# mit-han-lab/pvcnn

Hardware: AMD Instinct MI355X
Metric: point-clouds/sec fwd+bwd, PVCNN S3DIS N=4096 R=32 (higher is better)
Workload: dtype f32 (fp32 tensors, fp32 accumulate; Conv3d fwd / bwd-data / bwd-weight and the large SharedMLP fwd / bwd-data / bwd-weight products as power-of-two scaled fp16 hi+lo splits, 3 partial products on fp16 MFMA, max rel err vs fp64 1e-6 <= the fp32-MFMA kernels'; PVCNN_CONV_MATH=fp32 PVCNN_PW_MATH=fp32 s; 1 GPU; PVCNN (1xC) S3DIS fwd+bwd+Adam, B=16/GPU N=4096 R=32/16 fp32; global_batch=16, points=4096, parallelism=dp1, gradient_bytes=10289972, step_mode=graph, rccl_ranks=0, gradient_buckets=2

## Files before the change

### include/pvcnn_hip.h

```cpp
#ifndef PVCNN_HIP_H_
#define PVCNN_HIP_H_

#include <stddef.h>
#include <stdint.h>

#ifdef __cplusplus
extern "C" {
#endif

#if defined(__GNUC__)
#define PVCNN_API __attribute__((visibility("default")))
#else
#define PVCNN_API
#endif

#define PVCNN_ABI_VERSION 15
#define PVCNN_OK 0
#define PVCNN_ERR_INVALID_ARGUMENT (-1)

PVCNN_API int pvcnn_version(void);
PVCNN_API const char *pvcnn_last_error_string(void);

PVCNN_API int pvcnn_voxel_coords(const float *coords, int B, int N, int R, int normalize, float eps, float *norm_coords,
                       int32_t *vox_coords, void *stream);

PVCNN_API int pvcnn_voxel_coords_tail(const float *coords, long coords_batch_stride, const float *mean, const float *radius,
                            int B, int N, int R, float eps, float *norm_coords, int32_t *vox_coords, void *stream);

PVCNN_API size_t pvcnn_avg_voxelize_fwd_workspace_bytes(int B, int C, int N, int R);
PVCNN_API int pvcnn_avg_voxelize_fwd(const float *feat, const int32_t *coords, int B, int C, int N, int R,
                           float *out, int32_t *ind, int32_t *cnt, void *workspace,
                           size_t workspace_bytes, void *stream);
PVCNN_API int pvcnn_avg_voxelize_bwd(const float *grad_y, const int32_t *ind, const int32_t *cnt, int B,
                           int C, int N, int S, float *grad_x, void *stream);

PVCNN_API int pvcnn_trilinear_devox_fwd(const float *coords, const float *feat, int B, int C, int N, int R,
                              int is_training, int32_t *inds, float *wgts, float *outs,
                              void *stream);
PVCNN_API size_t pvcnn_trilinear_devox_bwd_workspace_bytes(int B, int C, int N, int R);
PVCNN_API int pvcnn_trilinear_devox_bwd(const float *grad_y, const int32_t *inds, const float *wgts, int B,
                              int C, int N, int R, float *grad_x, void *workspace,
                              size_t workspace_bytes, void *stream);

PVCNN_API size_t pvcnn_avg_voxelize_plan_bytes(int B, int N, int R);
PVCNN_API size_t pvcnn_avg_voxelize_plan_scratch_bytes(int B, int N, int R);
PVCNN_API int pvcnn_avg_voxelize_plan(const int32_t *coords, int B, int N, int R, int32_t *ind, int32_t *cnt, void *plan,
                            size_t plan_bytes, void *scratch, size_t scratch_bytes, void *stream);
PVCNN_API size_t pvcnn_pvconv_plans_scratch_bytes(int B, int N, int R);
PVCNN_API int pvcnn_pvconv_plans(const int32_t *vox_coords, const float *norm_coords, int B, int N, int R, int32_t *ind, int32_t *cnt,
                                 void *vox_plan, size_t vox_plan_bytes, void *devox_bwd_plan, size_t devox_bwd_plan_bytes,
                                 void *scratch, size_t scratch_bytes, void *stream);
PVCNN_API int pvcnn_avg_voxelize_apply(const float *feat, const void *plan, size_t plan_bytes, int B, int C, int N, int R,
                             float *out, void *stream);
PVCNN_API size_t pvcnn_trilinear_devox_bwd_plan_bytes(int B, int N, int R);
PVCNN_API size_t pvcnn_trilinear_devox_bwd_plan_scratch_bytes(int B, int N, int R);
PVCNN_API int pvcnn_trilinear_devox_bwd_plan(const int32_t *inds, const float *wgts, int B, int N, int R, void *plan,
                                   size_t plan_bytes, void *scratch, size_t scratch_bytes, void *stream);
PVCNN_API int pvcnn_trilinear_devox_bwd_apply(const float *grad_y, long grad_y_batch_stride, const void *plan, size_t plan_bytes,
                                    int B, int C, int N, int R, float *grad_x, void *stream);

PVCNN_API int pvcnn_ball_query(const float *centers, const float *points, int B, int N, int M, float radius,
                     int U, int32_t *out, void *stream);

PVCNN_API int pvcnn_grouping_fwd(const float *features, const int32_t *indices, int B, int C, int N, int M,
                       int U, float *out, void *stream);
PVCNN_API size_t pvcnn_grouping_bwd_workspace_bytes(int B, int C, int N, int M, int U);
PVCNN_API int pvcnn_grouping_bwd(const float *grad_y, const int32_t *indices, int B, int C, int N, int M,
                       int U, float *grad_x, void *workspace, size_t workspace_bytes, void *stream);
PVCNN_API int pvcnn_gather_fwd(const float *features, const int32_t *indices, int B, int C, int N, int M,
                     float *out, void *stream);
PVCNN_API size_t pvcnn_gather_bwd_workspace_bytes(int B, int C, int N, int M);
PVCNN_API int pvcnn_gather_bwd(const float *grad_y, const int32_t *indices, int B, int C, int N, int M,
                     float *grad_x, void *workspace, size_t workspace_bytes, void *stream);

#define PVCNN_FPS_MAX_RESIDENT_POINTS 16384
PVCNN_API int pvcnn_fps(const float *coords, int B, int N, int M, float *distances, int32_t *indices,
              void *stream);

PVCNN_API int pvcnn_mask_select(const uint8_t *mask, int B, int N, int M, const int32_t *choices, const int64_t *seed,
                      int32_t *selected, int32_t *count, void *stream);

PVCNN_API size_t pvcnn_batch_lds_bytes(int N, int max_n);
PVCNN_API int pvcnn_batch_s3dis(const float *rows, const void *labels, int label_bytes, const int64_t *offsets, long long W, int max_n,
                      const int64_t *order, long long order_len, const int64_t *cursor, int B, int N, int C_out,
// ... 202 lines not shown
```

### pvcnn_amd/__init__.py

```python
import importlib
import sys

__version__ = '0.1.0'

_DROPIN_SUBMODULES = (
    'ball_query', 'frustum', 'loss', 'pointnet', 'pvconv', 'se', 'shared_mlp', 'voxelization',
    'functional', 'functional.backend', 'functional.ball_query', 'functional.devoxelization',
    'functional.grouping', 'functional.interpolatation', 'functional.loss', 'functional.sampling',
    'functional.voxelization',
)


def install_dropin(name='modules'):
    impl = importlib.import_module('pvcnn_amd.modules')
    sys.modules[name] = impl
    for sub in _DROPIN_SUBMODULES:
        sys.modules[f'{name}.{sub}'] = importlib.import_module(f'pvcnn_amd.modules.{sub}')
    return impl


_ADOPTED = {}


def _adopted_class(cls, forward, extra=None):
# ... 24 lines not shown
    from .modules import SharedMLP

    def is_head(seq):
        kids = list(seq)
        return (len(kids) >= 2 and isinstance(kids[0], SharedMLP) and isinstance(kids[-1], (nn.Conv1d, SharedMLP))
                and all(isinstance(k, (SharedMLP, nn.Dropout, nn.Conv1d)) for k in kids))

    def take(module, donor_forward, extra=None):
        if type(module).forward is not donor_forward:
            module.__class__ = _adopted_class(type(module), donor_forward, extra)

    for m in model.modules():
        if type(m) is nn.Sequential and is_head(m):
            m.__class__ = _adopted_class(nn.Sequential, _classify_forward)
    has = lambda obj, *names: all(hasattr(obj, a) for a in names)
    if has(model, 'inst_seg_net', 'center_reg_net', 'box_est_net'):
        seg, ctr, box = model.inst_seg_net, model.center_reg_net, model.box_est_net
        if has(seg, 'point_features', 'cloud_features', 'classifier', 'in_channels'):
            take(seg, workload._FrustumSegmentation.forward)
        if has(ctr, 'features', 'regression'):
            take(ctr, workload._CloudRegressor.forward, {'_head_attr': 'regression', '_coords_tuple': False})
        if has(box, 'features', 'classifier'):
            take(box, workload._CloudRegressor.forward, {'_head_attr': 'classifier', '_coords_tuple': True})
        return model
    donor = None
    if has(model, 'sa_layers', 'fp_layers', 'classifier'):
        donor = workload.PVCNN2
    elif has(model, 'point_features', 'classifier', 'num_shapes', 'in_channels') and isinstance(model.point_features, nn.ModuleList):
        donor = workload.PVCNNShapeNet
    elif has(model, 'point_features', 'cloud_features', 'classifier') and isinstance(model.point_features, nn.ModuleList):
        donor = workload.PVCNN
    if donor is not None:
        take(model, donor.forward)
    return model
```

### pvcnn_amd/_lib.py

```python
import ctypes
import functools
import os

import torch

_CSRC = os.path.join(os.path.dirname(os.path.abspath(__file__)), 'csrc')
LIB_PATH = os.path.join(_CSRC, 'libpvcnn_hip.so')
ABI_VERSION = 15

_vp, _i, _f, _sz, _l = ctypes.c_void_p, ctypes.c_int, ctypes.c_float, ctypes.c_size_t, ctypes.c_long
_ll = ctypes.c_longlong

SIGNATURES = {
    'pvcnn_version': (_i, []),
    'pvcnn_last_error_string': (ctypes.c_char_p, []),
    'pvcnn_voxel_coords': (_i, [_vp, _i, _i, _i, _i, _f, _vp, _vp, _vp]),
    'pvcnn_voxel_coords_tail': (_i, [_vp, ctypes.c_long, _vp, _vp, _i, _i, _i, _f, _vp, _vp, _vp]),
    'pvcnn_avg_voxelize_fwd_workspace_bytes': (_sz, [_i, _i, _i, _i]),
    'pvcnn_avg_voxelize_fwd': (_i, [_vp, _vp, _i, _i, _i, _i, _vp, _vp, _vp, _vp, _sz, _vp]),
    'pvcnn_avg_voxelize_bwd': (_i, [_vp, _vp, _vp, _i, _i, _i, _i, _vp, _vp]),
    'pvcnn_trilinear_devox_fwd': (_i, [_vp, _vp, _i, _i, _i, _i, _i, _vp, _vp, _vp, _vp]),
    'pvcnn_trilinear_devox_bwd_workspace_bytes': (_sz, [_i, _i, _i, _i]),
    'pvcnn_trilinear_devox_bwd': (_i, [_vp, _vp, _vp, _i, _i, _i, _i, _vp, _vp, _sz, _vp]),
    'pvcnn_avg_voxelize_plan_bytes': (_sz, [_i, _i, _i]),
    'pvcnn_avg_voxelize_plan_scratch_bytes': (_sz, [_i, _i, _i]),
    'pvcnn_avg_voxelize_plan': (_i, [_vp, _i, _i, _i, _vp, _vp, _vp, _sz, _vp, _sz, _vp]),
    'pvcnn_avg_voxelize_apply': (_i, [_vp, _vp, _sz, _i, _i, _i, _i, _vp, _vp]),
    'pvcnn_pvconv_plans_scratch_bytes': (_sz, [_i, _i, _i]),
    'pvcnn_pvconv_plans': (_i, [_vp, _vp, _i, _i, _i, _vp, _vp, _vp, _sz, _vp, _sz, _vp, _sz, _vp]),
    'pvcnn_trilinear_devox_bwd_plan_bytes': (_sz, [_i, _i, _i]),
    'pvcnn_trilinear_devox_bwd_plan_scratch_bytes': (_sz, [_i, _i, _i]),
    'pvcnn_trilinear_devox_bwd_plan': (_i, [_vp, _vp, _i, _i, _i, _vp, _sz, _vp, _sz, _vp]),
    'pvcnn_trilinear_devox_bwd_apply': (_i, [_vp, ctypes.c_long, _vp, _sz, _i, _i, _i, _i, _vp, _vp]),
    'pvcnn_ball_query': (_i, [_vp, _vp, _i, _i, _i, _f, _i, _vp, _vp]),
    'pvcnn_grouping_fwd': (_i, [_vp, _vp, _i, _i, _i, _i, _i, _vp, _vp]),
    'pvcnn_grouping_bwd_workspace_bytes': (_sz, [_i, _i, _i, _i, _i]),
    'pvcnn_grouping_bwd': (_i, [_vp, _vp, _i, _i, _i, _i, _i, _vp, _vp, _sz, _vp]),
    'pvcnn_gather_fwd': (_i, [_vp, _vp, _i, _i, _i, _i, _vp, _vp]),
    'pvcnn_gather_bwd_workspace_bytes': (_sz, [_i, _i, _i, _i]),
    'pvcnn_gather_bwd': (_i, [_vp, _vp, _i, _i, _i, _i, _vp, _vp, _sz, _vp]),
    'pvcnn_fps': (_i, [_vp, _i, _i, _i, _vp, _vp, _vp]),
    'pvcnn_mask_select': (_i, [_vp, _i, _i, _i, _vp, _vp, _vp, _vp, _vp]),
    'pvcnn_three_nn_interp_fwd': (_i, [_vp, _vp, _vp, _i, _i, _i, _i, _vp, _vp, _vp, _vp]),
    'pvcnn_three_nn_interp_bwd_workspace_bytes': (_sz, [_i, _i, _i, _i]),
    'pvcnn_three_nn_interp_bwd': (_i, [_vp, _vp, _vp, _i, _i, _i, _i, _vp, _vp, _sz, _vp]),
    'pvcnn_conv3d_weight_transform': (_i, [_vp, _i, _i, _i, _vp, _vp]),
    'pvcnn_conv3d_fwd': (_i, [_vp, _vp, _vp, _i, _i, _i, _i, _vp, _vp]),
    'pvcnn_conv3d_bwd_weight_workspace_bytes': (_sz, [_i, _i, _i, _i]),
    'pvcnn_conv3d_bwd_weight': (_i, [_vp, _vp, _i, _i, _i, _i, _vp, _vp, _vp, _sz, _vp]),
    'pvcnn_conv3d_weight_split_bytes': (_sz, [_i, _i, _i, _i]),
    'pvcnn_conv3d_weight_split': (_i, [_vp, _i, _i, _i, _i, _vp, _vp]),
    'pvcnn_conv3d_weight_split_pair': (_i, [_vp, _i, _i, _vp, _vp, _vp]),
    'pvcnn_conv3d_fwd_split_stats_parts': (_sz, [_i, _i, _i, _i]),
    'pvcnn_conv3d_fwd_split_route': (_i, [_i, _i, _i, _i, _i]),
    'pvcnn_absmax_bits': (_i, [_vp, _sz, _vp, _vp]),
    'pvcnn_absmax_tiles_count': (_sz, [_i, ctypes.c_long, _i]),
    'pvcnn_absmax_tiles': (_i, [_vp, _i, _i, ctypes.c_long, _i, _vp, _vp, _vp]),
    'pvcnn_conv3d_bwd_weight_f16_workspace_bytes': (_sz, [_i, _i, _i, _i]),
    'pvcnn_conv3d_bwd_weight_f16': (_i, [_vp, _vp, _vp, _i, _vp, _i, _i, _i, _i, _i, _vp, _vp, _vp, _sz, _vp]),
    'pvcnn_conv3d_fwd_split': (_i, [_vp, _vp, _vp, _i, _i, _i, _i, _i, _vp, _i, _vp, _vp, _vp]),
    'pvcnn_pwconv_transpose': (_i, [_vp, _i, _i, _vp, _vp]),
    'pvcnn_pwconv_fwd': (_i, [_vp, _vp, _i, _vp, _i, _i, _i, _i, _vp, _vp]),
# ... 113 lines not shown
```

### pvcnn_amd/csrc/csr.h

```cpp
#pragma once
#include <algorithm>

#include "slab.h"

namespace pvcnn {

constexpr int kCsrThreads = 1024;
constexpr int kCsrMaxTargets = 1 << 20;
constexpr int kCsrMaxRange = 14336;

__host__ __device__ __forceinline__ int pad32(int v) { return v + (v >> 5); }
__host__ __device__ __forceinline__ int start_stride(int L) { return (L + 1 + 3) & ~3; }

constexpr int kTileTargets = 4096;
constexpr int kTileThreads = 1024;
__host__ __device__ inline int order_stride(int L) { return ceil_div(L, kTileTargets) * kTileTargets; }

constexpr int kGroupSlack = 256;
__host__ __device__ inline long entw_range_base(int start_t0, int r) { return 2L * start_t0 + (long)r * (kTileTargets / kWave) * kGroupSlack; }
__host__ __device__ inline long entw_stride(int L, long E) { return 2L * E + (long)ceil_div(L, kTileTargets) * (kTileTargets / kWave) * kGroupSlack; }

struct CsrPlan {
  int32_t *start;
  int2 *ent;
// ... 716 lines not shown
template <class EP1, class EP2>
int launch_csr_prep_pair(const EP1 &ep1, long E1_, int32_t *cnt1, void *plan1, size_t plan1_bytes, const EP2 &ep2, long E2_, void *plan2,
                         size_t plan2_bytes, int B, int L, void *scratch, size_t scratch_bytes, hipStream_t s, const char *what) {
  const int E1 = (int)E1_, E2 = (int)E2_;
  if (B == 0) return 0;
  const size_t s1 = csr_prep_scratch_bytes(B, E1), s2 = csr_prep_scratch_bytes(B, E2);
  if (!plan1 || !plan2 || plan1_bytes < CsrPlan::bytes(B, L, E1) || plan2_bytes < CsrPlan::bytes(B, L, E2) || !aligned16(plan1) ||
      !aligned16(plan2) || !scratch || !aligned16(scratch) || scratch_bytes < s1 + s2) {
    set_error("%s: plans / scratch missing, misaligned or too small (%zu, %zu, %zu bytes needed)", what, CsrPlan::bytes(B, L, E1),
              CsrPlan::bytes(B, L, E2), s1 + s2);
    return PVCNN_ERR_INVALID_ARGUMENT;
  }
  CsrPlan p1, p2;
  p1.carve(plan1, B, L, E1);
  p2.carve(plan2, B, L, E2);
  const int total = std::max(2, std::min(16, kNumCU / std::max(B, 1)));
  const int cap1 = std::max(1, total / 4);
  const CsrSplit sp1 = csr_split(B, L, E1, cap1), sp2 = csr_split(B, L, E2, std::max(1, total - cap1));
  const size_t prep_lds = ((size_t)kCsrCoarse * 2 + 4 + 32 + 4 + 3 * kCsrList + std::max(sp1.HP, sp2.HP)) * sizeof(int);
  auto k = csr_prep_pair_kernel<EP1, EP2>;
  if (int e = enable_big_lds(k, prep_lds)) { set_error("%s: LDS attribute: %d", what, e); return e; }
  char *sc = static_cast<char *>(scratch);
  hipLaunchKernelGGL(k, dim3(sp1.P + sp2.P, B), dim3(kCsrThreads), prep_lds, s, ep1, E1, sp1, cnt1, p1.start, reinterpret_cast<int32_t *>(sc),
                     p1.ent, ep2, E2, sp2, p2.start, reinterpret_cast<int32_t *>(sc + s1), p2.ent, L);
  if (int e = check_launch(what)) return e;
  const CsrPlanRef r1{p1.start, p1.ent, p1.order, p1.seg, p1.gofs, p1.entw, E1}, r2{p2.start, p2.ent, p2.order, p2.seg, p2.gofs, p2.entw, E2};
  const int nr = ceil_div(L, kTileTargets), nblk = order_stride(L) / 256;
  hipLaunchKernelGGL(csr_order_pair_kernel, dim3(2 * nr, B), dim3(kTileThreads), 0, s, r1, r2, L, nr);
  if (int e = check_launch(what)) return e;
  hipLaunchKernelGGL(csr_interleave_pair_kernel, dim3(2 * nblk, B), dim3(256), 0, s, r1, r2, L, nblk);
  return check_launch(what);
}

inline int launch_csr_apply(const float *src, const void *plan, size_t plan_bytes, float *dst, int B, int C, int L, int J, long E_,
                            hipStream_t s, const char *what, long src_bstride = 0) {
  if (src_bstride <= 0) src_bstride = (long)C * J;
  const int E = (int)E_;
  if (B == 0 || C == 0) return 0;
  if (!plan || plan_bytes < CsrPlan::bytes(B, L, E) || !aligned16(plan)) {
    set_error("%s: plan missing, misaligned or too small (%zu bytes needed)", what, CsrPlan::bytes(B, L, E));
    return PVCNN_ERR_INVALID_ARGUMENT;
  }
  CsrPlan pl;
  pl.carve(const_cast<void *>(plan), B, L, E);
  const int JP = (J + 3) & ~3;
  int G = 0;
  for (int cand = 4; cand >= 1; cand >>= 1)
    if ((size_t)cand * (JP + kTileTargets) * sizeof(float) <= (size_t)kLdsBytesPerCU) { G = cand; break; }
  const size_t row = (size_t)J * sizeof(float);
  int GS = 1;
  if (row > 0 && row <= 64 * 1024) {
    GS = (int)std::min<size_t>(8, (64 * 1024) / row);
    while (GS > 1 && (long)B * ceil_div(C, GS) < 2L * kNumCU) GS >>= 1;
    if (GS >= 8) GS = 8; else if (GS >= 4) GS = 4; else if (GS >= 2) GS = 2; else GS = 1;
  }
  const bool very_sparse = (long)E * 4 <= (long)L && row > 0 && row <= (size_t)kLdsBytesPerCU && (long)B * ceil_div(C, GS) >= kNumCU;
  if (G > 0 && J > 0 && !very_sparse) {
    while (G > 1 && G / 2 >= C) G >>= 1;
    const int nr = ceil_div(L, kTileTargets), slabs = ceil_div(C, G);
    int nsplit = 1;
    while (nsplit < nr && (long)B * slabs * nsplit < kNumCU) nsplit <<= 1;
    nsplit = std::min(nsplit, nr);
    const size_t lds = (size_t)G * (JP + kTileTargets) * sizeof(float);
    const dim3 grid(slabs, nsplit, B);
#define PVCNN_TILE(GV)                                                                                                   \
  do {                                                                                                                   \
// ... 38 lines not shown
```

### pvcnn_amd/csrc/voxelize.hip

```cpp
#include <algorithm>

#include "csr.h"

namespace pvcnn {

__global__ __launch_bounds__(256) void vox_stats_atomic_kernel(const int32_t *__restrict__ coords, int N,
                                                               int R, int S, int32_t *__restrict__ ind,
                                                               int32_t *__restrict__ cnt) {
  const int b = blockIdx.y, i = blockIdx.x * 256 + threadIdx.x;
  if (i >= N) return;
  const int32_t *co = coords + (size_t)b * 3 * N;
  int v = co[i] * R * R + co[i + N] * R + co[i + 2 * N];
  v = min(max(v, 0), S - 1);
  ind[(size_t)b * N + i] = v;
  atomicAdd(cnt + (size_t)b * S + v, 1);
}

__global__ __launch_bounds__(256) void vox_scatter_atomic_kernel(
    const float *__restrict__ feat, const int32_t *__restrict__ ind, const int32_t *__restrict__ cnt, int C,
    int N, int S, int CT, float *__restrict__ out) {
  const int b = blockIdx.z, i = blockIdx.x * 256 + threadIdx.x;
  if (i >= N) return;
  const int pos = ind[(size_t)b * N + i];
  const int cur = cnt[(size_t)b * S + pos];
// ... 198 lines not shown
  PVCNN_REQUIRE(B >= 0 && N >= 0 && R > 0, "negative size");
  PVCNN_REQUIRE((long)R * R * R <= 0x7fffffffL / 4, "resolution too large");
  const int S = R * R * R;
  if (B == 0) return 0;
  PVCNN_REQUIRE(csr_supported(S, N), "grid too large for a plan: use pvcnn_avg_voxelize_fwd");
  PVCNN_REQUIRE(cnt && (ind || N == 0) && (coords || N == 0), "null pointer");
  PVCNN_REQUIRE(B <= 65535, "batch > 65535");
  VoxelEntries ep{coords, ind, N, R, S};
  return launch_csr_prep(ep, B, S, N, cnt, plan, plan_bytes, scratch, scratch_bytes, static_cast<hipStream_t>(stream),
                         "avg_voxelize_plan");
}

extern "C" size_t pvcnn_pvconv_plans_scratch_bytes(int B, int N, int R) {
  if (B <= 0 || N < 0 || R <= 0) return 0;
  return csr_prep_scratch_bytes(B, N) + csr_prep_scratch_bytes(B, 8L * N);
}

extern "C" int pvcnn_pvconv_plans(const int32_t *vox_coords, const float *norm_coords, int B, int N, int R, int32_t *ind, int32_t *cnt,
                                  void *vox_plan, size_t vox_plan_bytes, void *devox_bwd_plan, size_t devox_bwd_plan_bytes, void *scratch,
                                  size_t scratch_bytes, void *stream) {
  PVCNN_REQUIRE(B >= 0 && N > 0 && R > 0, "bad size");
  PVCNN_REQUIRE((long)R * R * R <= 0x7fffffffL / 4, "resolution too large");
  const int S = R * R * R;
  if (B == 0) return 0;
  PVCNN_REQUIRE(csr_supported(S, 8L * N), "grid too large for a plan: use the one-shot calls");
  PVCNN_REQUIRE(cnt && ind && vox_coords && norm_coords, "null pointer");
  PVCNN_REQUIRE(B <= 65535, "batch > 65535");
  VoxelEntries e1{vox_coords, ind, N, R, S};
  CoordTapEntries e2{norm_coords, N, R, R * R, S};
  return launch_csr_prep_pair(e1, N, cnt, vox_plan, vox_plan_bytes, e2, 8L * N, devox_bwd_plan, devox_bwd_plan_bytes, B, S,
                              scratch, scratch_bytes, static_cast<hipStream_t>(stream), "pvconv_plans");
}

extern "C" int pvcnn_avg_voxelize_apply(const float *feat, const void *plan, size_t plan_bytes, int B, int C, int N, int R,
                                        float *out, void *stream) {
  PVCNN_REQUIRE(B >= 0 && C >= 0 && N >= 0 && R > 0, "negative size");
  PVCNN_REQUIRE((long)R * R * R <= 0x7fffffffL / 4, "resolution too large");
  if (B == 0 || C == 0) return 0;
  PVCNN_REQUIRE(out && (feat || N == 0), "null pointer");
  PVCNN_REQUIRE(B <= 65535, "batch > 65535");
  const int S = R * R * R;
  return launch_csr_apply(feat, plan, plan_bytes, out, B, C, S, N, N, static_cast<hipStream_t>(stream),
                          "avg_voxelize_apply");
}
```

### pvcnn_amd/modules/functional/backend.py

```python
import ctypes
import os

import torch

from ... import _lib
from . import _cache

__all__ = ['_backend']


def _dev(t, name):
    if not t.is_cuda:
        raise RuntimeError(f'{name} must be a CUDA (HIP) tensor -- the PVConv hot path has no CPU implementation')


def _f32(t, name):
    _dev(t, name)
    if not t.is_contiguous():
        raise RuntimeError(f'{name} must be a contiguous tensor')
    if t.dtype != torch.float32:
        raise RuntimeError(f'{name} must be a float tensor')


def _f32_rows(t, name):
# ... 364 lines not shown
        vp.r, vp.n, vp.b = r, n, b
        vp.ind = torch.empty((b, n), dtype=torch.int32, device=dev)
        vp.cnt = torch.empty((b, r * r * r), dtype=torch.int32, device=dev)
        vp.plan = torch.empty((nbytes,), dtype=torch.uint8, device=dev)
        scratch = self._scratch(self.lib.pvcnn_avg_voxelize_plan_scratch_bytes(b, n, r), dev)
        with _Launch(coords) as s:
            _lib.check(self.lib.pvcnn_avg_voxelize_plan(_p(coords), b, n, r, _p(vp.ind), _p(vp.cnt), _p(vp.plan), vp.plan.numel(),
                                                        _p(scratch), scratch.numel(), s), 'avg_voxelize_plan')
        return vp

    has_pvconv_plans = os.environ.get('PVCNN_PAIR_PLANS', '1') != '0'

    def pvconv_plans(self, vox_coords, norm_coords, resolution):
        _i32(vox_coords, 'vox_coords'); _f32(norm_coords, 'norm_coords')
        _shape(vox_coords.dim() == 3 and vox_coords.shape[1] == 3 and tuple(norm_coords.shape) == tuple(vox_coords.shape),
               'pvconv_plans: vox_coords / norm_coords (B,3,N) expected')
        b, _, n = vox_coords.shape
        r = int(resolution)
        vbytes, dbytes = self.lib.pvcnn_avg_voxelize_plan_bytes(b, n, r), self.lib.pvcnn_trilinear_devox_bwd_plan_bytes(b, n, r)
        if vbytes == 0 or dbytes == 0 or n == 0:
            return None
        dev = vox_coords.device
        vp = self.VoxelPlan()
        vp.r, vp.n, vp.b = r, n, b
        vp.ind = torch.empty((b, n), dtype=torch.int32, device=dev)
        vp.cnt = torch.empty((b, r * r * r), dtype=torch.int32, device=dev)
        vp.plan = torch.empty((vbytes,), dtype=torch.uint8, device=dev)
        dplan = torch.empty((dbytes,), dtype=torch.uint8, device=dev)
        scratch = self._scratch(self.lib.pvcnn_pvconv_plans_scratch_bytes(b, n, r), dev)
        with _Launch(vox_coords) as s:
            _lib.check(self.lib.pvcnn_pvconv_plans(_p(vox_coords), _p(norm_coords), b, n, r, _p(vp.ind), _p(vp.cnt), _p(vp.plan), vp.plan.numel(),
                                                   _p(dplan), dplan.numel(), _p(scratch), scratch.numel(), s), 'pvconv_plans')
        return vp, dplan

    def avg_voxelize_apply(self, features, vp):
        _f32(features, 'features')
        _shape(features.dim() == 3 and features.shape[0] == vp.b and features.shape[2] == vp.n, 'avg_voxelize: features do not match the plan')
        b, c, n = features.shape
        out = torch.empty((b, c, vp.r ** 3), dtype=torch.float32, device=features.device)
        with _Launch(features) as s:
            _lib.check(self.lib.pvcnn_avg_voxelize_apply(_p(features), _p(vp.plan), vp.plan.numel(), b, c, n, vp.r, _p(out), s),
                       'avg_voxelize_apply')
        return out

    def trilinear_devoxelize_backward_plan(self, indices, weights, r):
        _i32(indices, 'indices'); _f32(weights, 'weights')
        _shape(indices.dim() == 3 and indices.shape[1] == 8 and indices.shape == weights.shape, 'inds / wgts (B,8,N) expected')
        b, _, n = indices.shape
        r = int(r)
        nbytes = self.lib.pvcnn_trilinear_devox_bwd_plan_bytes(b, n, r)
        if nbytes == 0:
            return None
        plan = torch.empty((nbytes,), dtype=torch.uint8, device=indices.device)
        scratch = self._scratch(self.lib.pvcnn_trilinear_devox_bwd_plan_scratch_bytes(b, n, r), indices.device)
        with _Launch(indices) as s:
            _lib.check(self.lib.pvcnn_trilinear_devox_bwd_plan(_p(indices), _p(weights), b, n, r, _p(plan), plan.numel(),
                                                               _p(scratch), scratch.numel(), s), 'trilinear_devoxelize_backward_plan')
        return plan

    def trilinear_devoxelize_backward_apply(self, grad_y, plan, r):
        gy_bstride = _f32_rows(grad_y, 'grad_y')
        b, c, n = grad_y.shape
        r = int(r)
        grad_x = torch.empty((b, c, r * r * r), dtype=torch.float32, device=grad_y.device)
        with _Launch(grad_y) as s:
            _lib.check(self.lib.pvcnn_trilinear_devox_bwd_apply(_p(grad_y), gy_bstride, _p(plan), plan.numel(), b, c, n, r,
# ... 995 lines not shown
```

### pvcnn_amd/modules/voxelization.py

```python
import torch
import torch.nn as nn

from . import functional as F
from .functional import _cache
from .functional._autograd import native

__all__ = ['Voxelization']


class Voxelization(nn.Module):
    single_launch = False

    def __init__(self, resolution, normalize=True, eps=0):
        super().__init__()
        self.r = int(resolution)
        self.normalize = normalize
        self.eps = eps

    def normalized_coords(self, coords):
        centred = coords.detach()
        centred = centred - centred.mean(2, keepdim=True)
        if self.normalize:
            radius = centred.norm(dim=1, keepdim=True).max(dim=2, keepdim=True).values
            unit = centred / (radius * 2.0 + self.eps) + 0.5
        else:
            unit = (centred + 1) / 2.0
        return torch.clamp(unit * self.r, 0, self.r - 1)

    @staticmethod
    def _statistics(coords, normalize):
        c = coords.detach()
        mean = c.mean(2, keepdim=True)
        radius = None
        if normalize:
            radius = (c - mean).norm(dim=1, keepdim=True).max(dim=2, keepdim=True).values
        return mean, radius

    def grid_coordinates(self, coords):
        be = native()
        normalize = bool(self.normalize)
        if self.single_launch:
            return self._fresh(coords, ('vox1', self.r, normalize, float(self.eps)),
                               lambda: be.voxel_coords(coords.detach().contiguous(), self.r, normalize, self.eps))

        def tail():
            mean, radius = _cache.memo(coords, ('stats', normalize), lambda: self._statistics(coords, normalize))
            c = coords.detach()
            from .functional.backend import batch_strided_ok
            if not batch_strided_ok(c):
                c = c.contiguous()
            return be.voxel_coords_tail(c, mean.contiguous(), radius.contiguous() if radius is not None else None, self.r, self.eps)
        return self._fresh(coords, ('vox', self.r, normalize, float(self.eps)), tail)

    @staticmethod
    def _fresh(coords, key, make):
        def stamped():
            norm, vox = make()
            return norm, vox, norm._version, vox._version
        for _ in range(2):
            norm, vox, vn, vv = _cache.memo(coords, key, stamped)
            if norm._version == vn and vox._version == vv:
                return norm, vox
            _cache.forget(coords, key)
        return norm, vox

    def forward(self, features, coords):
        be = native()
        if coords.is_cuda and coords.dtype == torch.float32 and coords.dim() == 3 and getattr(be, 'has_voxel_coords', False):
            norm_coords, vox_coords = self.grid_coordinates(coords)
            if getattr(be, 'has_pvconv_plans', False) and torch.is_grad_enabled() and self.training:
                self._plan_pair(be, norm_coords, vox_coords)
        else:
            norm_coords = self.normalized_coords(coords)
            vox_coords = torch.round(norm_coords).to(torch.int32)
        return F.avg_voxelize(features, vox_coords, self.r), norm_coords

    def _plan_pair(self, be, norm_coords, vox_coords):
        from .functional import _cache
        from .functional.devoxelization import CornerTaps
        built = []

        def make():
            pair = be.pvconv_plans(vox_coords, norm_coords.contiguous(), self.r) if norm_coords.is_contiguous() and vox_coords.is_contiguous() else None
            if pair is None:
                return be.avg_voxelize_plan(vox_coords.contiguous(), self.r)
            built.append(pair[1])
            return pair[0]
        _cache.memo(vox_coords, ('avg_voxelize_plan', self.r), make)
        if built:
            taps = CornerTaps.of(norm_coords, self.r)
            if taps.plan is None:
                taps.plan = built[0]

    def extra_repr(self):
        tail = f', normalized eps = {self.eps}' if self.normalize else ''
        return f'resolution={self.r}{tail}'
```

### pvcnn_amd/workload.py

```python
import contextlib

import torch
import torch.nn as nn

from .modules import PVConv, PointNetAModule, PointNetFPModule, PointNetSAModule, SharedMLP
from .modules.functional.bnact import emit_row_max, run_layers
from .modules.functional.dense import run_dense

SEED = 1588147245

__all__ = ['PVCNN', 'PVCNN2', 'PVCNNShapeNet', 'FrustumPVCNNE', 'make_s3dis_batch', 'make_shapenet_batch',
           'make_frustum_batch', 'make_frustum_targets', 'frustum_size_templates', 'SEED']


def _scaled(width, k):
    return int(k * width)


class _TapAndPool(torch.autograd.Function):

    @staticmethod
    def forward(ctx, x, winners, values=None):
        ctx.save_for_backward(winners)
        ctx.npoints = x.shape[-1]
        return x.view_as(x), (values.view_as(values) if values is not None else x.gather(2, winners.unsqueeze(-1)).squeeze(-1))

    @staticmethod
    def backward(ctx, g_tap, g_pool):
        (winners,) = ctx.saved_tensors
        if g_tap is None and g_pool is None:
            return None, None, None
        if g_tap is None:
            g = torch.zeros(g_pool.shape + (int(ctx.npoints),), dtype=g_pool.dtype, device=g_pool.device)
        elif getattr(g_tap, '_pvcnn_private_slice', False) and not torch.is_grad_enabled():
            g = g_tap
        else:
            g = g_tap.clone(memory_format=torch.contiguous_format)
        if g_pool is not None:
# ... 156 lines not shown
    if classify:
        layers.append(nn.Conv1d(cin, last, 1) if pointwise else nn.Linear(cin, last))
        return layers, last
    layers.append(block(cin, _scaled(last, width)))
    return layers, _scaled(last, width)


def _pv_stack(cin, spec, width, vres, **pvconv_kw):
    cout, repeat, res = spec
    cout = _scaled(cout, width)
    blocks = []
    for _ in range(repeat):
        if res is None:
            blocks.append(SharedMLP(cin, cout))
        else:
            blocks.append(PVConv(cin, cout, kernel_size=3, resolution=int(vres * res), **pvconv_kw))
        cin = cout
    return blocks, cout


class PVCNN(nn.Module):
    blocks = ((64, 1, 32), (64, 2, 16), (128, 1, 16), (1024, 1, None))

    def __init__(self, num_classes, extra_feature_channels=6, width_multiplier=1, voxel_resolution_multiplier=1):
        super().__init__()
        self.in_channels = extra_feature_channels + 3
        stages, cin, concat = [], self.in_channels, 0
        for spec in self.blocks:
            blocks, cin = _pv_stack(cin, spec, width_multiplier, voxel_resolution_multiplier,
                                    with_se=False, normalize=True, eps=0)
            stages += blocks
            concat += cin * len(blocks)
        self.point_features = nn.ModuleList(stages)
        layers, c_cloud = _head(cin, [256, 128], width_multiplier, pointwise=False, classify=False)
        self.cloud_features = nn.Sequential(*layers)
        layers, _ = _head(concat + c_cloud, [512, 0.3, 256, 0.3, num_classes], width_multiplier,
                          pointwise=True, classify=True)
        self.classifier = nn.Sequential(*layers)

    def forward(self, inputs):
        if isinstance(inputs, dict):
            inputs = inputs['features']
        coords = inputs[:, :3, :]
        feats, taps = inputs, []
        last = len(self.point_features) - 1
        slot = slot_amax = None
        for i, stage in enumerate(self.point_features):
            if i == last:
                slot = concat_slot(taps, _out_channels(stage), _in_channels(self.classifier), feats, self.training)
            with (emit_row_max(_last_norm(stage), out=slot.view if slot is not None else None) if i == last else contextlib.nullcontext()):
                feats, _ = stage((feats, coords))
            taps.append(feats)
        if slot is not None and slot.holds(feats):
            slot_amax = _amax_tag(feats)
        taps[-1], pooled = tap_and_pool(feats)
        cloud = run_dense(self.cloud_features, pooled)
        taps.append(cloud.unsqueeze(-1).expand(-1, -1, coords.size(-1)))
        return _classify(self.classifier, concat_points(taps, slot, slot_amax))


_CENTERS_AHEAD = __import__('os').environ.get('PVCNN_CENTERS_AHEAD', '1') != '0'
_CENTERS_AHEAD_LEVELS = int(__import__('os').environ.get('PVCNN_CENTERS_AHEAD_LEVELS', '0'))
_side_streams = {}


class _SamplingChain:
# ... 101 lines not shown
        if isinstance(inputs, dict):
            inputs = inputs['features']
        coords, feats = inputs[:, :3, :].contiguous(), inputs
        coords_pyramid, skips = [], []
        ahead = centers_ahead(self.sa_layers, coords)
        try:
            for stage in self.sa_layers:
                skips.append(feats)
                coords_pyramid.append(coords)
                feats, coords = stage((feats, coords))
        finally:
            for sa in ahead or ():
                sa.__dict__.pop('_centers_ahead', None)
        skips[0] = inputs[:, 3:, :].contiguous()
        for i, stage in enumerate(self.fp_layers):
            feats, coords = stage((coords_pyramid[-1 - i], coords, feats, skips[-1 - i]))
        return _classify(self.classifier, feats)


class PVCNNShapeNet(nn.Module):
    blocks = ((64, 1, 32), (128, 2, 16), (512, 1, None), (2048, 1, None))

    def __init__(self, num_classes, num_shapes, extra_feature_channels=3, width_multiplier=1, voxel_resolution_multiplier=1):
        super().__init__()
        self.in_channels = extra_feature_channels + 3
        self.num_shapes = num_shapes
        stages, cin, concat = [], self.in_channels, 0
        for spec in self.blocks:
            blocks, cin = _pv_stack(cin, spec, width_multiplier, voxel_resolution_multiplier,
                                    with_se=True, normalize=False, eps=0)
            stages += blocks
            concat += cin * len(blocks)
        self.point_features = nn.ModuleList(stages)
        layers, _ = _head(num_shapes + cin + concat, [256, 0.2, 256, 0.2, 128, num_classes], width_multiplier,
                          pointwise=True, classify=True)
        self.classifier = nn.Sequential(*layers)

    def forward(self, inputs):
        feats = inputs[:, :self.in_channels, :]
        taps = [inputs[:, -self.num_shapes:, :]]
        coords = feats[:, :3, :]
        last = len(self.point_features) - 1
        slot = slot_amax = None
        for i, stage in enumerate(self.point_features):
            if i == last:
                slot = concat_slot(taps, _out_channels(stage), _in_channels(self.classifier), feats, self.training)
            with (emit_row_max(_last_norm(stage), out=slot.view if slot is not None else None) if i == last else contextlib.nullcontext()):
                feats, _ = stage((feats, coords))
            taps.append(feats)
        if slot is not None and slot.holds(feats):
            slot_amax = _amax_tag(feats)
        taps[-1], pooled = tap_and_pool(feats)
        taps.append(pooled.unsqueeze(-1).expand(-1, -1, coords.size(-1)))
        return _classify(self.classifier, concat_points(taps, slot, slot_amax))


class _FrustumSegmentation(nn.Module):
    point_blocks = ((64, 2, 16), (64, 1, 12), (128, 1, 12), (1024, 1, None))

    def __init__(self, num_classes, extra_feature_channels, width_multiplier, voxel_resolution_multiplier):
        super().__init__()
        self.in_channels = extra_feature_channels + 3
        self.num_classes = num_classes
        stages, cin = [], self.in_channels
        for spec in self.point_blocks:
            blocks, cin = _pv_stack(cin, spec, width_multiplier, voxel_resolution_multiplier, with_se=False)
# ... 163 lines not shown
```

Measured before the change: 2568 point-clouds/s.

## Build voxelize and devox plans for all resolutions in one batched launch set

Adds a multi-level plan builder that prepares the voxelization and devoxelization-backward CSR plans for every distinct voxel resolution (32 and 16 here) in a single set of three kernel launches, instead of one launch set per level. Level tables are passed by value, and each block picks its level from a prefix offset. Voxelization modules that share normalization settings are grouped, so the first stage builds plans for all levels and later stages find them in the memo cache. The aim is fewer launches and better GPU fill for small per-level grids, in exchange for more complex dispatch and all plans being built up front.

```diff
diff --git a/include/pvcnn_hip.h b/include/pvcnn_hip.h
--- a/include/pvcnn_hip.h
+++ b/include/pvcnn_hip.h
@@ -14,7 +14,7 @@
 #define PVCNN_API
 #endif
 
-#define PVCNN_ABI_VERSION 15
+#define PVCNN_ABI_VERSION 16
 #define PVCNN_OK 0
 #define PVCNN_ERR_INVALID_ARGUMENT (-1)
 
@@ -50,6 +50,10 @@
 PVCNN_API int pvcnn_pvconv_plans(const int32_t *vox_coords, const float *norm_coords, int B, int N, int R, int32_t *ind, int32_t *cnt,
                                  void *vox_plan, size_t vox_plan_bytes, void *devox_bwd_plan, size_t devox_bwd_plan_bytes,
                                  void *scratch, size_t scratch_bytes, void *stream);
+PVCNN_API int pvcnn_pvconv_plans_multi(const int32_t *const *vox_coords, const float *const *norm_coords, int B, int N, const int *R,
+                                       int nlevels, int32_t *const *ind, int32_t *const *cnt, void *const *vox_plan,
+                                       const size_t *vox_plan_bytes, void *const *devox_bwd_plan, const size_t *devox_bwd_plan_bytes,
+                                       void *scratch, size_t scratch_bytes, void *stream);
 PVCNN_API int pvcnn_avg_voxelize_apply(const float *feat, const void *plan, size_t plan_bytes, int B, int C, int N, int R,
                              float *out, void *stream);
 PVCNN_API size_t pvcnn_trilinear_devox_bwd_plan_bytes(int B, int N, int R);
diff --git a/pvcnn_amd/__init__.py b/pvcnn_amd/__init__.py
--- a/pvcnn_amd/__init__.py
+++ b/pvcnn_amd/__init__.py
@@ -80,4 +80,7 @@
         donor = workload.PVCNN
     if donor is not None:
         take(model, donor.forward)
+        if donor is not workload.PVCNN2:
+            from .modules.voxelization import Voxelization
+            Voxelization.share_plan_levels(model.point_features)
     return model
diff --git a/pvcnn_amd/_lib.py b/pvcnn_amd/_lib.py
--- a/pvcnn_amd/_lib.py
+++ b/pvcnn_amd/_lib.py
@@ -6,7 +6,7 @@
 
 _CSRC = os.path.join(os.path.dirname(os.path.abspath(__file__)), 'csrc')
 LIB_PATH = os.path.join(_CSRC, 'libpvcnn_hip.so')
-ABI_VERSION = 15
+ABI_VERSION = 16
 
 _vp, _i, _f, _sz, _l = ctypes.c_void_p, ctypes.c_int, ctypes.c_float, ctypes.c_size_t, ctypes.c_long
 _ll = ctypes.c_longlong
@@ -28,6 +28,7 @@
     'pvcnn_avg_voxelize_apply': (_i, [_vp, _vp, _sz, _i, _i, _i, _i, _vp, _vp]),
     'pvcnn_pvconv_plans_scratch_bytes': (_sz, [_i, _i, _i]),
     'pvcnn_pvconv_plans': (_i, [_vp, _vp, _i, _i, _i, _vp, _vp, _vp, _sz, _vp, _sz, _vp, _sz, _vp]),
+    'pvcnn_pvconv_plans_multi': (_i, [_vp, _vp, _i, _i, _vp, _i, _vp, _vp, _vp, _vp, _vp, _vp, _vp, _sz, _vp]),
     'pvcnn_trilinear_devox_bwd_plan_bytes': (_sz, [_i, _i, _i]),
     'pvcnn_trilinear_devox_bwd_plan_scratch_bytes': (_sz, [_i, _i, _i]),
     'pvcnn_trilinear_devox_bwd_plan': (_i, [_vp, _vp, _i, _i, _i, _vp, _sz, _vp, _sz, _vp]),
diff --git a/pvcnn_amd/csrc/csr.h b/pvcnn_amd/csrc/csr.h
--- a/pvcnn_amd/csrc/csr.h
+++ b/pvcnn_amd/csrc/csr.h
@@ -772,6 +772,160 @@
   return check_launch(what);
 }
 
+constexpr int kCsrMaxLevels = 4;
+
+template <class EP1, class EP2>
+struct CsrPrepLevel {
+  EP1 ep1;
+  EP2 ep2;
+  CsrSplit sp1, sp2;
+  int32_t *cnt1, *start1, *tmp1;
+  int2 *ent1;
+  int32_t *start2, *tmp2;
+  int2 *ent2;
+  int E1, E2, L;
+  int first;
+};
+template <class EP1, class EP2>
+struct CsrPrepTable {
+  CsrPrepLevel<EP1, EP2> lv[kCsrMaxLevels];
+  int n;
+};
+
+template <class EP1, class EP2>
+__global__ __launch_bounds__(kCsrThreads) void csr_prep_multi_kernel(CsrPrepTable<EP1, EP2> t) {
+  extern __shared__ __attribute__((aligned(16))) int csr_lds[];
+  int p = (int)blockIdx.x, l = 0;
+#pragma unroll
+  for (int i = 1; i < kCsrMaxLevels; ++i)
+    if (i < t.n && p >= t.lv[i].first) l = i;
+  const CsrPrepLevel<EP1, EP2> &lv = t.lv[l];
+  p -= lv.first;
+  if (p < lv.sp1.P) {
+    const EP1 ep = lv.ep1;
+    const CsrSplit sp = lv.sp1;
+    csr_prep_body(ep, lv.E1, lv.L, sp, lv.cnt1, lv.start1, lv.tmp1, lv.ent1, p, (int)blockIdx.y, csr_lds);
+  } else {
+    const EP2 ep = lv.ep2;
+    const CsrSplit sp = lv.sp2;
+    csr_prep_body(ep, lv.E2, lv.L, sp, static_cast<int32_t *>(nullptr), lv.start2, lv.tmp2, lv.ent2, p - lv.sp1.P, (int)blockIdx.y, csr_lds);
+  }
+}
+
+struct CsrOrderLevel {
+  CsrPlanRef a, c;
+  int L;
+  int n;
+  int first;
+};
+struct CsrOrderTable {
+  CsrOrderLevel lv[kCsrMaxLevels];
+  int n;
+};
+
+[[maybe_unused]] static __global__ __launch_bounds__(kTileThreads) void csr_order_multi_kernel(CsrOrderTable t) {
+  int r = (int)blockIdx.x, l = 0;
+#pragma unroll
+  for (int i = 1; i < kCsrMaxLevels; ++i)
+    if (i < t.n && r >= t.lv[i].first) l = i;
+  const CsrOrderLevel &lv = t.lv[l];
+  r -= lv.first;
+  const bool f = r < lv.n;
+  const CsrPlanRef pr = f ? lv.a : lv.c;
+  csr_order_body(pr.start, pr.ent, lv.L, pr.E, pr.order, pr.seg, pr.gofs, pr.entw, f ? r : r - lv.n, (int)blockIdx.y);
+}
+
+[[maybe_unused]] static __global__ __launch_bounds__(256) void csr_interleave_multi_kernel(CsrOrderTable t) {
+  int k = (int)blockIdx.x, l = 0;
+#pragma unroll
+  for (int i = 1; i < kCsrMaxLevels; ++i)
+    if (i < t.n && k >= t.lv[i].first) l = i;
+  const CsrOrderLevel &lv = t.lv[l];
+  k -= lv.first;
+  const bool f = k < lv.n;
+  const CsrPlanRef pr = f ? lv.a : lv.c;
+  csr_interleave_body(pr.ent, pr.seg, pr.gofs, lv.L, pr.E, pr.entw, f ? k : k - lv.n, (int)blockIdx.y);
+}
+
+template <class EP1, class EP2>
+struct CsrPairArgs {
+  EP1 ep1;
+  long E1;
+  int32_t *cnt1;
+  void *plan1;
+  size_t plan1_bytes;
+  EP2 ep2;
+  long E2;
+  void *plan2;
+  size_t plan2_bytes;
+  int L;
+};
+
+template <class EP1, class EP2>
+int launch_csr_prep_multi(const CsrPairArgs<EP1, EP2> *levels, int nlevels, int B, void *scratch, size_t scratch_bytes, hipStream_t s,
+                          const char *what) {
+  if (B == 0 || nlevels == 0) return 0;
+  if (nlevels < 0 || nlevels > kCsrMaxLevels) {
+    set_error("%s: 1..%d levels expected", what, kCsrMaxLevels);
+    return PVCNN_ERR_INVALID_ARGUMENT;
+  }
+  size_t need = 0;
+  for (int l = 0; l < nlevels; ++l) {
+    const auto &a = levels[l];
+    if (!a.plan1 || !a.plan2 || a.plan1_bytes < CsrPlan::bytes(B, a.L, a.E1) || a.plan2_bytes < CsrPlan::bytes(B, a.L, a.E2) ||
+        !aligned16(a.plan1) || !aligned16(a.plan2)) {
+      set_error("%s: plans of level %d missing, misaligned or too small (%zu, %zu bytes needed)", what, l, CsrPlan::bytes(B, a.L, a.E1),
+                CsrPlan::bytes(B, a.L, a.E2));
+      return PVCNN_ERR_INVALID_ARGUMENT;
+    }
+    need += csr_prep_scratch_bytes(B, a.E1) + csr_prep_scratch_bytes(B, a.E2);
+  }
+  if (!scratch || !aligned16(scratch) || scratch_bytes < need) {
+    set_error("%s: scratch missing, misaligned or too small (%zu bytes needed)", what, need);
+    return PVCNN_ERR_INVALID_ARGUMENT;
+  }
+  const int total = std::max(2, std::min(16, kNumCU / std::max(B, 1)));
+  const int cap1 = std::max(1, total / 4);
+  CsrPrepTable<EP1, EP2> pt{};
+  CsrOrderTable ot{}, it{};
+  pt.n = ot.n = it.n = nlevels;
+  int first_p = 0, first_r = 0, first_k = 0, hp = 0;
+  char *sc = static_cast<char *>(scratch);
+  for (int l = 0; l < nlevels; ++l) {
+    const auto &a = levels[l];
+    const int E1 = (int)a.E1, E2 = (int)a.E2;
+    CsrPlan p1, p2;
+    p1.carve(a.plan1, B, a.L, E1);
+    p2.carve(a.plan2, B, a.L, E2);
+    auto &q = pt.lv[l];
+    q.ep1 = a.ep1; q.ep2 = a.ep2;
+    q.sp1 = csr_split(B, a.L, E1, cap1);
+    q.sp2 = csr_split(B, a.L, E2, std::max(1, total - cap1));
+    q.cnt1 = a.cnt1; q.start1 = p1.start; q.ent1 = p1.ent;
+    q.start2 = p2.start; q.ent2 = p2.ent;
+    q.tmp1 = reinterpret_cast<int32_t *>(sc); sc += csr_prep_scratch_bytes(B, E1);
+    q.tmp2 = reinterpret_cast<int32_t *>(sc); sc += csr_prep_scratch_bytes(B, E2);
+    q.E1 = E1; q.E2 = E2; q.L = a.L;
+    q.first = first_p;
+    first_p += q.sp1.P + q.sp2.P;
+    hp = std::max(hp, std::max(q.sp1.HP, q.sp2.HP));
+    const CsrPlanRef r1{p1.start, p1.ent, p1.order, p1.seg, p1.gofs, p1.entw, E1}, r2{p2.start, p2.ent, p2.order, p2.seg, p2.gofs, p2.entw, E2};
+    ot.lv[l] = CsrOrderLevel{r1, r2, a.L, ceil_div(a.L, kTileTargets), first_r};
+    it.lv[l] = CsrOrderLevel{r1, r2, a.L, order_stride(a.L) / 256, first_k};
+    first_r += 2 * ot.lv[l].n;
+    first_k += 2 * it.lv[l].n;
+  }
+  const size_t prep_lds = ((size_t)kCsrCoarse * 2 + 4 + 32 + 4 + 3 * kCsrList + hp) * sizeof(int);
+  auto k = csr_prep_multi_kernel<EP1, EP2>;
+  if (int e = enable_big_lds(k, prep_lds)) { set_error("%s: LDS attribute: %d", what, e); return e; }
+  hipLaunchKernelGGL(k, dim3(first_p, B), dim3(kCsrThreads), prep_lds, s, pt);
+  if (int e = check_launch(what)) return e;
+  hipLaunchKernelGGL(csr_order_multi_kernel, dim3(first_r, B), dim3(kTileThreads), 0, s, ot);
+  if (int e = check_launch(what)) return e;
+  hipLaunchKernelGGL(csr_interleave_multi_kernel, dim3(first_k, B), dim3(256), 0, s, it);
+  return check_launch(what);
+}
+
 inline int launch_csr_apply(const float *src, const void *plan, size_t plan_bytes, float *dst, int B, int C, int L, int J, long E_,
                             hipStream_t s, const char *what, long src_bstride = 0) {
   if (src_bstride <= 0) src_bstride = (long)C * J;
diff --git a/pvcnn_amd/csrc/voxelize.hip b/pvcnn_amd/csrc/voxelize.hip
--- a/pvcnn_amd/csrc/voxelize.hip
+++ b/pvcnn_amd/csrc/voxelize.hip
@@ -254,6 +254,30 @@
                               scratch, scratch_bytes, static_cast<hipStream_t>(stream), "pvconv_plans");
 }
 
+extern "C" int pvcnn_pvconv_plans_multi(const int32_t *const *vox_coords, const float *const *norm_coords, int B, int N, const int *R,
+                                        int nlevels, int32_t *const *ind, int32_t *const *cnt, void *const *vox_plan,
+                                        const size_t *vox_plan_bytes, void *const *devox_bwd_plan, const size_t *devox_bwd_plan_bytes,
+                                        void *scratch, size_t scratch_bytes, void *stream) {
+  PVCNN_REQUIRE(B >= 0 && N > 0, "bad size");
+  PVCNN_REQUIRE(nlevels >= 1 && nlevels <= kCsrMaxLevels, "1..4 levels expected");
+  PVCNN_REQUIRE(vox_coords && norm_coords && R && ind && cnt && vox_plan && vox_plan_bytes && devox_bwd_plan && devox_bwd_plan_bytes,
+                "null table");
+  if (B == 0) return 0;
+  PVCNN_REQUIRE(B <= 65535, "batch > 65535");
+  CsrPairArgs<VoxelEntries, CoordTapEntries> lv[kCsrMaxLevels];
+  for (int l = 0; l < nlevels; ++l) {
+    const int r = R[l];
+    PVCNN_REQUIRE(r > 0 && (long)r * r * r <= 0x7fffffffL / 4, "resolution out of range");
+    const int S = r * r * r;
+    PVCNN_REQUIRE(csr_supported(S, 8L * N), "grid too large for a plan: use the one-shot calls");
+    PVCNN_REQUIRE(cnt[l] && ind[l] && vox_coords[l] && norm_coords[l], "null pointer");
+    lv[l] = CsrPairArgs<VoxelEntries, CoordTapEntries>{VoxelEntries{vox_coords[l], ind[l], N, r, S}, N, cnt[l], vox_plan[l], vox_plan_bytes[l],
+                                                       CoordTapEntries{norm_coords[l], N, r, r * r, S}, 8L * N, devox_bwd_plan[l],
+                                                       devox_bwd_plan_bytes[l], S};
+  }
+  return launch_csr_prep_multi(lv, nlevels, B, scratch, scratch_bytes, static_cast<hipStream_t>(stream), "pvconv_plans_multi");
+}
+
 extern "C" int pvcnn_avg_voxelize_apply(const float *feat, const void *plan, size_t plan_bytes, int B, int C, int N, int R,
                                         float *out, void *stream) {
   PVCNN_REQUIRE(B >= 0 && C >= 0 && N >= 0 && R > 0, "negative size");
diff --git a/pvcnn_amd/modules/functional/backend.py b/pvcnn_amd/modules/functional/backend.py
--- a/pvcnn_amd/modules/functional/backend.py
+++ b/pvcnn_amd/modules/functional/backend.py
@@ -420,6 +420,42 @@
             _lib.check(self.lib.pvcnn_pvconv_plans(_p(vox_coords), _p(norm_coords), b, n, r, _p(vp.ind), _p(vp.cnt), _p(vp.plan), vp.plan.numel(),
                                                    _p(dplan), dplan.numel(), _p(scratch), scratch.numel(), s), 'pvconv_plans')
         return vp, dplan
+
+    has_pvconv_plans_multi = os.environ.get('PVCNN_MULTI_PLANS', '1') != '0'
+    max_plan_levels = 4
+
+    def pvconv_plans_multi(self, vox_coords, norm_coords, resolutions):
+        import ctypes
+        levels = len(resolutions)
+        _shape(1 <= levels <= self.max_plan_levels and len(vox_coords) == levels and len(norm_coords) == levels,
+               f'pvconv_plans_multi: 1..{self.max_plan_levels} levels expected')
+        b, _, n = vox_coords[0].shape
+        for vox, norm in zip(vox_coords, norm_coords):
+            _i32(vox, 'vox_coords'); _f32(norm, 'norm_coords')
+            _shape(tuple(vox.shape) == (b, 3, n) and tuple(norm.shape) == (b, 3, n), 'pvconv_plans_multi: vox_coords / norm_coords (B,3,N) expected')
+        rs = [int(r) for r in resolutions]
+        sizes = [(self.lib.pvcnn_avg_voxelize_plan_bytes(b, n, r), self.lib.pvcnn_trilinear_devox_bwd_plan_bytes(b, n, r)) for r in rs]
+        if n == 0 or any(v == 0 or d == 0 for v, d in sizes):
+            return None
+        dev = vox_coords[0].device
+        out = []
+        for r, (vbytes, dbytes) in zip(rs, sizes):
+            vp = self.VoxelPlan()
+            vp.r, vp.n, vp.b = r, n, b
+            vp.ind = torch.empty((b, n), dtype=torch.int32, device=dev)
+            vp.cnt = torch.empty((b, r * r * r), dtype=torch.int32, device=dev)
+            vp.plan = torch.empty((vbytes,), dtype=torch.uint8, device=dev)
+            out.append((vp, torch.empty((dbytes,), dtype=torch.uint8, device=dev)))
+        scratch = self._scratch(sum(self.lib.pvcnn_pvconv_plans_scratch_bytes(b, n, r) for r in rs), dev)
+        ptrs = lambda tensors: (ctypes.c_void_p * levels)(*[t.data_ptr() for t in tensors])
+        sizes_of = lambda tensors: (ctypes.c_size_t * levels)(*[t.numel() for t in tensors])
+        with _Launch(vox_coords[0]) as s:
+            _lib.check(self.lib.pvcnn_pvconv_plans_multi(ptrs(vox_coords), ptrs(norm_coords), b, n, (ctypes.c_int * levels)(*rs), levels,
+                                                         ptrs([vp.ind for vp, _ in out]), ptrs([vp.cnt for vp, _ in out]),
+                                                         ptrs([vp.plan for vp, _ in out]), sizes_of([vp.plan for vp, _ in out]),
+                                                         ptrs([d for _, d in out]), sizes_of([d for _, d in out]),
+                                                         _p(scratch), scratch.numel(), s), 'pvconv_plans_multi')
+        return out
 
     def avg_voxelize_apply(self, features, vp):
         _f32(features, 'features')
diff --git a/pvcnn_amd/modules/voxelization.py b/pvcnn_amd/modules/voxelization.py
--- a/pvcnn_amd/modules/voxelization.py
+++ b/pvcnn_amd/modules/voxelization.py
@@ -10,6 +10,7 @@
 
 class Voxelization(nn.Module):
     single_launch = False
+    plan_levels = ()
 
     def __init__(self, resolution, normalize=True, eps=0):
         super().__init__()
@@ -36,12 +37,13 @@
             radius = (c - mean).norm(dim=1, keepdim=True).max(dim=2, keepdim=True).values
         return mean, radius
 
-    def grid_coordinates(self, coords):
+    def grid_coordinates(self, coords, r=None):
         be = native()
+        r = self.r if r is None else int(r)
         normalize = bool(self.normalize)
         if self.single_launch:
-            return self._fresh(coords, ('vox1', self.r, normalize, float(self.eps)),
-                               lambda: be.voxel_coords(coords.detach().contiguous(), self.r, normalize, self.eps))
+            return self._fresh(coords, ('vox1', r, normalize, float(self.eps)),
+                               lambda: be.voxel_coords(coords.detach().contiguous(), r, normalize, self.eps))
 
         def tail():
             mean, radius = _cache.memo(coords, ('stats', normalize), lambda: self._statistics(coords, normalize))
@@ -49,8 +51,8 @@
             from .functional.backend import batch_strided_ok
             if not batch_strided_ok(c):
                 c = c.contiguous()
-            return be.voxel_coords_tail(c, mean.contiguous(), radius.contiguous() if radius is not None else None, self.r, self.eps)
-        return self._fresh(coords, ('vox', self.r, normalize, float(self.eps)), tail)
+            return be.voxel_coords_tail(c, mean.contiguous(), radius.contiguous() if radius is not None else None, r, self.eps)
+        return self._fresh(coords, ('vox', r, normalize, float(self.eps)), tail)
 
     @staticmethod
     def _fresh(coords, key, make):
@@ -69,11 +71,33 @@
         if coords.is_cuda and coords.dtype == torch.float32 and coords.dim() == 3 and getattr(be, 'has_voxel_coords', False):
             norm_coords, vox_coords = self.grid_coordinates(coords)
             if getattr(be, 'has_pvconv_plans', False) and torch.is_grad_enabled() and self.training:
+                if len(self.plan_levels) > 1 and getattr(be, 'has_pvconv_plans_multi', False) and _cache.enabled:
+                    self._plan_levels(be, coords)
                 self._plan_pair(be, norm_coords, vox_coords)
         else:
             norm_coords = self.normalized_coords(coords)
             vox_coords = torch.round(norm_coords).to(torch.int32)
         return F.avg_voxelize(features, vox_coords, self.r), norm_coords
+
+    def _plan_levels(self, be, coords):
+        from .functional.devoxelization import CornerTaps
+        levels = tuple(self.plan_levels)
+        key = ('pvconv_plans_multi', levels, bool(self.normalize), float(self.eps), bool(self.single_launch))
+
+        def make():
+            grids = [self.grid_coordinates(coords, r) for r in levels]
+            if not all(norm.is_contiguous() and vox.is_contiguous() for norm, vox in grids):
+                return False
+            pairs = be.pvconv_plans_multi([vox for _, vox in grids], [norm for norm, _ in grids], levels)
+            if pairs is None:
+                return False
+            for r, (norm, vox), (vp, dplan) in zip(levels, grids, pairs):
+                if _cache.memo(vox, ('avg_voxelize_plan', r), lambda vp=vp: vp) is vp:
+                    taps = CornerTaps.of(norm, r)
+                    if taps.plan is None:
+                        taps.plan = dplan
+            return True
+        _cache.memo(coords, key, make)
 
     def _plan_pair(self, be, norm_coords, vox_coords):
         from .functional import _cache
@@ -92,6 +116,17 @@
             if taps.plan is None:
                 taps.plan = built[0]
 
+    @staticmethod
+    def share_plan_levels(root, max_levels=4):
+        groups = {}
+        for m in root.modules():
+            if isinstance(m, Voxelization):
+                groups.setdefault((bool(m.normalize), float(m.eps)), []).append(m)
+        for members in groups.values():
+            levels = tuple(sorted({m.r for m in members}, reverse=True))
+            for m in members:
+                m.plan_levels = levels if 1 < len(levels) <= max_levels else ()
+
     def extra_repr(self):
         tail = f', normalized eps = {self.eps}' if self.normalize else ''
         return f'resolution={self.r}{tail}'
diff --git a/pvcnn_amd/workload.py b/pvcnn_amd/workload.py
--- a/pvcnn_amd/workload.py
+++ b/pvcnn_amd/workload.py
@@ -4,6 +4,7 @@
 import torch.nn as nn
 
 from .modules import PVConv, PointNetAModule, PointNetFPModule, PointNetSAModule, SharedMLP
+from .modules.voxelization import Voxelization
 from .modules.functional.bnact import emit_row_max, run_layers
 from .modules.functional.dense import run_dense
 
@@ -226,6 +227,7 @@
             stages += blocks
             concat += cin * len(blocks)
         self.point_features = nn.ModuleList(stages)
+        Voxelization.share_plan_levels(self.point_features)
         layers, c_cloud = _head(cin, [256, 128], width_multiplier, pointwise=False, classify=False)
         self.cloud_features = nn.Sequential(*layers)
         layers, _ = _head(concat + c_cloud, [512, 0.3, 256, 0.3, num_classes], width_multiplier,
@@ -393,6 +395,7 @@
             stages += blocks
             concat += cin * len(blocks)
         self.point_features = nn.ModuleList(stages)
+        Voxelization.share_plan_levels(self.point_features)
         layers, _ = _head(num_shapes + cin + concat, [256, 0.2, 256, 0.2, 128, num_classes], width_multiplier,
                           pointwise=True, classify=True)
         self.classifier = nn.Sequential(*layers)
```

Result: no change. 2567 point-clouds/s (-0.0%).
